# iceychris/LibreASR

Measured on AMD Instinct MI355X. Metric: audio-sec/sec/GPU (16 kHz streaming RNN-T) + p50 per-chunk latency, higher is better.
Workload: dtype f32

## Files before the change

libreasr_amd/csrc/lasr_ctx.hip.h:

```cpp
#pragma once
#include <dlfcn.h>

#include "lasr_results.hip.h"

constexpr int NW = 8;
constexpr int NCMD = 64;
constexpr int MTA = 4;

struct Cell {
    int I = 0;
    void *WxA = nullptr, *WhA = nullptr;
    void *WxC = nullptr, *WhC = nullptr;
    float *bias = nullptr, *rbias = nullptr;
    float *bn_s = nullptr, *bn_t = nullptr;
    float *h0 = nullptr, *c0 = nullptr;
    float *tab = nullptr;
};

struct lasr_ctx {
    lasr_model_desc d;
    int device = 0;
    hipStream_t stream = nullptr;
    std::string err;
    std::vector<void*> dev_allocs;
// ... 70 lines not shown
        size_t g_size = 0, ea_size = 0;
    };
    hipStream_t stream_nb = nullptr; unsigned long long* nb_done = nullptr; float* nb_buf = nullptr; size_t nb_floats = 0;
    int nb_kind = 0, nb_wgs = 0; double nb_ms = 0.0;
    hipStream_t stream_dec = nullptr;
    hipStream_t stream_lm = nullptr;
    hipEvent_t ev_lm_fork = nullptr, ev_lm_join = nullptr;
    double lm_stream_ratio[2] = {0.0, 0.0};
    int dec_stream_attempts = 0;
    double dec_stream_ratio = 0.0;
    static constexpr int NFLY = 32;
    static constexpr int RING = 64;
    static constexpr int TOKRING = 512, ENDSLOTS = 32;
    hipEvent_t ev_enc[NFLY] = {};
    hipEvent_t ev_misc = nullptr;
    int* T_row_ring[NFLY] = {};
    float* pe_ring = nullptr;
    int *c_cur = nullptr, *c_avail = nullptr, *c_iters = nullptr, *c_target = nullptr, *c_ntotal = nullptr;
    int* c_hcur_dev = nullptr;
    int *c_ntok_end = nullptr, *c_tok_ring = nullptr, *c_behind = nullptr, *c_enc_frames = nullptr, *c_enc_base = nullptr;
    int *c_done = nullptr, *c_flag_dev = nullptr;
    int* c_done2 = nullptr;
    int* c_iter = nullptr;
    std::map<std::tuple<int, int, int>, hipGraphExec_t> cgraphs;
    int* cont_host = nullptr;
    struct PendingStep { std::vector<int> rows; int Tm; int idx; bool admitted; std::vector<int> target; const int* T_row_ptr; long long serial;
                         std::vector<long long> frame_off; };
    std::vector<PendingStep> pending;
    std::vector<long long> h_frames_sub, h_fetched;
    std::vector<int> h_avail;
    std::vector<int> h_cur_seen;
    int work_left = 0;
    long long model_steps = 0, cont_iters = 0, iters_reported = 0;
    bool group_inflight = false;
    bool dec_tail_open = false;
    std::mutex mu;
    std::condition_variable cv_pump;
    std::condition_variable cv_prog;
    std::thread pump_th;
    bool pump_started = false, pump_on = false;
    std::atomic<bool> pump_stop{false};
    int pump_G = 3;
    std::atomic<long long> kick{0}, progress{0};
    int pump_rc = 0; std::string pump_err;
    int kick_n = 3, wait_n = 1;
    std::map<std::tuple<int, int, int, int, int>, hipGraphExec_t> graphs;
    bool use_graphs = true;
    bool main_graph = false;
    hipStream_t stream_cap = nullptr;
    std::map<std::vector<unsigned long long>, hipGraphExec_t> mgraphs;
    int* T_row_main = nullptr;

    struct LM {
        bool on = false;
        int E = 0, H = 0, L = 0;
        float alpha = 0.1f, theta = 1.0f, min_val = -10.0f;
        std::vector<Cell> cells;
        void* Wout = nullptr; float* bout = nullptr;
        float *ones = nullptr, *zeros = nullptr;
        std::vector<void*> h[2], y[2];
        std::vector<float*> cst[2];
        int par = 0;
        float *raw = nullptr, *lmz[2] = {nullptr, nullptr};
        int* valid[2] = {nullptr, nullptr};
        bool q8 = false;
        std::vector<void*> qWih, qWhh; void* qWout = nullptr;
        std::vector<float> s_ih, s_hh; float s_out = 0.f;
        std::vector<float*> b_ih, b_hh;
        std::vector<int> Kp_ih; int Kp_h = 0;
        float *gx = nullptr, *gh = nullptr;
        unsigned short* qa = nullptr; float* sx = nullptr;
        std::vector<unsigned short*> qh; std::vector<float*> sxh;
    } lm;

    struct Resampler { int U = 0, taps = 0, in_unit = 0; int* first = nullptr; float* w = nullptr; };
    std::map<int, Resampler> resamplers;

    int Tcap = 0;
    void *x0 = nullptr, *ybuf[2] = {nullptr, nullptr};
    float* pe_sync = nullptr;
    int tok_cap_alloc = 0;

    bool fe_fused = false;
    int ring_chunks = 0;
    std::vector<int> pend_serial;
    std::vector<char> pend_mat;
    float* win = nullptr; int* ring_pos = nullptr;
    float* pend = nullptr;
    float* stage_pcm = nullptr; size_t stage_pcm_floats = 0;
    float* win_rs = nullptr; size_t win_rs_floats = 0;
    static constexpr int NSTAGE = 64;
    hipEvent_t push_ev[NSTAGE] = {}; bool push_used[NSTAGE] = {};
    long long push_serial = 0;
    float* push_stage_host = nullptr;
    float* push_stage_host_dev = nullptr;
    float* push_stage_dev = nullptr;
    hipStream_t stream_copy = nullptr; hipEvent_t push_copied[NSTAGE] = {}; bool push_dma[NSTAGE] = {};
    struct CopyPool {
        bool init = false;
        std::vector<std::thread> th;
        std::mutex m; std::condition_variable cv;
        const char* src = nullptr; char* dst = nullptr; size_t bytes = 0, part_bytes = 0;
        const float* const* rows = nullptr; size_t row_bytes = 0;
        int parts = 0, next = 0, done = 0; long long gen = 0;
        std::atomic<long long> gen_hint{0}, done_hint{0};
        std::atomic<bool> stop{false};
    } pool;
    std::vector<int> h_ring_pos;
    struct LazyPush { bool on = false; const float* src = nullptr; std::vector<int> slots; int ev_i = -1; bool dma = false; } lazy;
    int pump_nap_pct = 0;
    int lazy_taken = 0, lazy_flushed = 0;
    bool lazy_on = true;
    float* lm_buf = nullptr; size_t lm_floats = 0;
    float* feat_stage = nullptr; size_t feat_stage_floats = 0;

    struct Cmd {
        int* T_row; int* what; int* src_idx; int* feat_sel; int* row_frames; int* token; int* emit;
        long long* row_N; long long* row_src_off; long long* row_feat_off;
    };
    char* cmd_host = nullptr; char* cmd_dev = nullptr; size_t cmd_bytes = 0; int cmd_next = 0; int cmd_inflight = 0;
    Cmd hc{}, dc{};

    int* res_host = nullptr;
    int* res_dev = nullptr;
    int* pub_arrivals = nullptr;
    size_t res_bytes = 0;

    std::vector<char> open_;
    std::vector<int> n_chunks, n_pend;
    std::vector<SlotResult> results;
    bool align_on = false;
    std::vector<long long> slot_frames;
    int* align_host = nullptr;
    int* c_frame_ring = nullptr; float* c_logp_ring = nullptr;
    struct Bias { int* block = nullptr; int n_nodes = 0; size_t n_edges = 0; bool has_back = false; int* node = nullptr; } bias;
    int* bias_pick_dev = nullptr;
    double* bias_round_dev = nullptr;

    static constexpr int NCELLEV = 64;
    bool cell_prof = false;
    bool cell_prof_events = true;
    hipEvent_t cp_ev[NCELLEV][2] = {};
    bool cp_ok = false;
    int cp_head = 0, cp_n = 0;
    int cp_cells[NCELLEV] = {};
    double cp_us = 0.0;
    long long cp_launches = 0;
    static constexpr int NCELLSLOT = 1 << 12;
    unsigned long long* cp_slots = nullptr;
    long long cp_slot_next = 0;
    std::vector<unsigned char> cp_slot_cells;
    int enc_wave = 0;
    double cp_clock_mhz = 100.0;

    static constexpr int NTRACE = 8192;
    bool tr_on = false;
    std::vector<hipEvent_t> tr_ev;
    std::vector<int> tr_tag;
    std::vector<double> tr_val;
    std::vector<int> tr_prev_cur, tr_prev_ntot;
    int tr_last_G = 0;
    hipEvent_t tr_base = nullptr;
    std::atomic<int> tr_n{0};

    struct Lattice {
        float* pp = nullptr; size_t pp_n = 0;
// ... 201 lines not shown
```

libreasr_amd/csrc/lasr_engine.hip:

```cpp
#include "lasr_host.hip.h"
#include <sys/prctl.h>
#include <time.h>

static void cont_poll(lasr_ctx* c);
static int cont_pump(lasr_ctx* c, int G);
static int pump_start(lasr_ctx* c);
static void pump_kick(lasr_ctx* c);
static int flush_lazy(lasr_ctx* c);
struct PushSrc;
static int submit_impl(lasr_ctx* c, const int* slots, int n, const PushSrc* fused, bool* fused_done);
static int push_submit_impl(lasr_ctx* c, const int* slots, int n, const float* pcm, int flags, long long* ticket, const float* const* rows);
static int overlap_probe_impl(lasr_ctx* c, int delay_us, double* ratio, hipStream_t sa = nullptr, hipStream_t sb = nullptr);
#include "lasr_prefix_tree.hip.h"
#include "lasr_bias.hip.h"
#include "lasr_cmd.hip.h"
#include "lasr_fe.hip.h"
#include "lasr_decode.hip.h"
#include "lasr_lattice_tables.hip.h"
#include "lasr_lattice.hip.h"
#include "lasr_lattice_post.hip.h"
#include "lasr_lattice_tree.hip.h"
#include "lasr_lm_score.hip.h"
#include "lasr_weights.hip.h"

// ... 248 lines not shown
            char* blk = nullptr;
            const size_t bytes = sizeof(double) * n_es + sizeof(int) * (n_tre + n_fd + n_ea) + 64;
            HIPCHK(c, hipHostMalloc((void**)&blk, bytes));
            c->host_allocs.push_back(blk);
            memset(blk, 0, bytes);
            void* dp = nullptr;
            HIPCHK(c, hipHostGetDevicePointer(&dp, blk, 0));
            char* dblk = (char*)dp;
            c->b_endsc_host = (double*)blk; c->b_endsc_dev = (double*)dblk;
            size_t off = sizeof(double) * n_es;
            c->b_tre_host = (int*)(blk + off); c->b_tre_dev = (int*)(dblk + off); off += sizeof(int) * n_tre;
            c->b_fdone_host = (int*)(blk + off); c->b_fdone_dev = (int*)(dblk + off); off += sizeof(int) * n_fd;
            c->b_endal_host = (int*)(blk + off); c->b_endal_dev = (int*)(dblk + off);
        }
    }
    RC(dalloc0(c, (char**)&c->ja, Mj * J * c->esz));
    RC(dalloc0(c, (char**)&c->cvt_a, (size_t)M * H * c->esz)); RC(dalloc0(c, (char**)&c->cvt_b, (size_t)M * H * c->esz));
    RC(dalloc0(c, &c->logits, Mj * V));
    RC(dalloc0(c, &c->ds.t_idx, M)); RC(dalloc0(c, &c->ds.iters, M)); RC(dalloc0(c, &c->ds.token, Md));
    RC(dalloc0(c, &c->ds.emit, Md)); RC(dalloc0(c, &c->ds.logp_sum, M));
    RC(dalloc0(c, &c->ds.sum_iters, M)); RC(dalloc0(c, &c->ds.n_ones, M)); RC(dalloc0(c, &c->zero_rows, M));
    RC(dalloc0(c, &c->pub_arrivals, 4));
    RC(dalloc0(c, &c->T_row_fix, M));
    RC(dalloc0(c, &c->T_row_main, M));
    {
        hipFuncAttributes fa{}, la_{};
        HIPCHK(c, hipFuncGetAttributes(&fa, (const void*)k_fe_mel<10>));
        HIPCHK(c, hipFuncGetAttributes(&la_, (const void*)k_logmel));
        const int lds_cu = 160 * 1024, excl = 98304;
        const bool wide_decode = c->Md >= 256 || lasr_ctx::LA_MAX * M >= 512;
        c->fe_lds_pad = wide_decode ? std::max(0, excl - (int)fa.sharedSizeBytes) : 0;
        if (getenv("LASR_FE_LDS_PAD")) c->fe_lds_pad = std::max(0, std::min(lds_cu - (int)fa.sharedSizeBytes, atoi(getenv("LASR_FE_LDS_PAD"))));
        c->logmel_lds_pad = c->fe_lds_pad ? std::max(0, excl - (int)la_.sharedSizeBytes) : 0;
        HIPCHK(c, hipFuncSetAttribute((const void*)k_fe_mel<10>, hipFuncAttributeMaxDynamicSharedMemorySize, lds_cu - (int)fa.sharedSizeBytes));
        HIPCHK(c, hipFuncSetAttribute((const void*)k_logmel, hipFuncAttributeMaxDynamicSharedMemorySize, lds_cu - (int)la_.sharedSizeBytes));
        HIPCHK(c, hipFuncSetAttribute((const void*)k_ln_tile, hipFuncAttributeMaxDynamicSharedMemorySize, 100 * 1024));
    }
    c->main_graph = c->bf != 0;
    if (getenv("LASR_MAIN_GRAPH")) c->main_graph = atoi(getenv("LASR_MAIN_GRAPH")) != 0;
    c->T_row_dev = c->zero_rows;
    for (int q = 0; q < lasr_ctx::NFLY; ++q) {
        RC(dalloc0(c, &c->T_row_ring[q], M));
        HIPCHK(c, hipEventCreateWithFlags(&c->ev_enc[q], hipEventDisableTiming));
    }
    HIPCHK(c, hipStreamCreateWithFlags(&c->stream_dec, hipStreamNonBlocking));
    HIPCHK(c, hipEventCreateWithFlags(&c->ev_misc, hipEventDisableTiming));
    {
        static const int pick = getenv("LASR_DEC_STREAM_PICK") ? atoi(getenv("LASR_DEC_STREAM_PICK")) : 1;
        std::vector<hipStream_t> rejected;
        c->dec_stream_attempts = 1;
        for (int attempt = 0; pick && attempt < 8; ++attempt) {
            double ratio = 0.0;
            if (overlap_probe_impl(c, 300, &ratio) != LASR_OK) { (void)hipGetLastError(); break; }
            c->dec_stream_ratio = ratio;
            if (ratio < 1.5) break;
            rejected.push_back(c->stream_dec);
            c->stream_dec = nullptr;
            HIPCHK(c, hipStreamCreateWithFlags(&c->stream_dec, hipStreamNonBlocking));
            c->dec_stream_attempts++;
        }
        for (hipStream_t st : rejected) (void)hipStreamDestroy(st);
        if (getenv("LASR_VERBOSE"))
            fprintf(stderr, "[lasr] decode stream: %d stream(s) tried, overlap probe %.2f\n", c->dec_stream_attempts, c->dec_stream_ratio);
    }
    RC(dalloc0(c, &c->pe_ring, (size_t)lasr_ctx::RING * M * J));
    RC(dalloc0(c, &c->c_cur, M)); RC(dalloc0(c, &c->c_avail, M)); RC(dalloc0(c, &c->c_iters, M)); RC(dalloc0(c, &c->c_target, M));
    RC(dalloc0(c, &c->c_ntotal, M)); RC(dalloc0(c, &c->c_enc_frames, M)); RC(dalloc0(c, &c->c_enc_base, M)); RC(dalloc0(c, &c->c_behind, 64));
    RC(dalloc0(c, &c->c_done, 64));
    RC(dalloc0(c, &c->c_done2, 64));
    RC(dalloc0(c, &c->c_iter, 4));
    HIPCHK(c, hipHostMalloc((void**)&c->cont_host, sizeof(int) * (16 + (size_t)M * (lasr_ctx::NFLY + lasr_ctx::ENDSLOTS + lasr_ctx::TOKRING))));
    memset(c->cont_host, 0, sizeof(int) * (16 + (size_t)M * (lasr_ctx::NFLY + lasr_ctx::ENDSLOTS + lasr_ctx::TOKRING)));
    {
        void* dp = nullptr;
        HIPCHK(c, hipHostGetDevicePointer(&dp, c->cont_host, 0));
        c->c_flag_dev = (int*)dp;
        c->c_hcur_dev = (int*)dp + 16;
        c->c_ntok_end = (int*)dp + 16 + (size_t)lasr_ctx::NFLY * M;
        c->c_tok_ring = c->c_ntok_end + (size_t)M * lasr_ctx::ENDSLOTS;
    }
    c->h_frames_sub.assign(M, 0); c->h_fetched.assign(M, 0); c->h_cur_seen.assign(M, 0); c->h_avail.assign(M, 0);
    c->fe_fused = M <= 512 && d.n_buffer <= 4 && d.n_stack == 10 && d.n_mels <= 128 && d.feat == 1280 && d.n_window + d.n_buffer - 1 <= 16
                  && !getenv("LASR_FE_LEGACY");
    c->h_ring_pos.assign(M, 0);
    c->ring_chunks = c->fe_fused ? d.n_window + d.n_buffer - 1 : d.n_window;
    c->pend_serial.assign((size_t)M * d.n_buffer, 0); c->pend_mat.assign((size_t)M * d.n_buffer, 0);
    RC(dalloc0(c, &c->win, (size_t)M * c->ring_chunks * d.chunk));
    RC(dalloc0(c, &c->ring_pos, M));
    RC(dalloc0(c, &c->pend, (size_t)M * d.n_buffer * d.n_stack * d.n_mels));

    lasr_ctx::Cmd tmp;
    c->cmd_bytes = cmd_layout(tmp, nullptr, M);
    HIPCHK(c, hipHostMalloc((void**)&c->cmd_host, c->cmd_bytes * NCMD));
    RC(dalloc0(c, &c->cmd_dev, c->cmd_bytes * NCMD));
    RC(ensure_T(c, std::max(d.n_buffer, 4)));

    {
        float* emb_dev = nullptr; float* EF = nullptr;
        RC(upload(c, &emb_dev, embed, (size_t)V * E));
        if (E != H) {
            Packed pk; void* wf = nullptr; float* bfn = nullptr;
            pack_tiles(pk, 0, H / 16, E, [&](int t, int ui, int k) { return ffn_w[(size_t)(16 * t + ui) * E + k]; });
            RC(upload_packed(c, &wf, pk)); RC(upload(c, &bfn, ffn_b, H));
            RC(dalloc(c, &EF, (size_t)V * H));
            GemmArgs g{}; set_operand(g, 0, emb_dev, E, 0, E / 16, wf); g.a_rows = V;
            EpiLinear::Args ea{}; ea.bias = bfn; ea.out = EF; ea.ldo = H; ea.n_rows = V; ea.t_idx = nullptr; ea.T_row = nullptr; ea.M = M;
            launch_table_gemm_f32(c, sync_view(c, c->la_sync), H / 16, V / 16, g, ea);
            HIPCHK(c, hipStreamSynchronize(c->stream));
            dfree(c, wf); dfree(c, bfn);
        } else {
            EF = emb_dev; emb_dev = nullptr;
        }
        const int G = c->G_pred;
        Packed pk; void* wt = nullptr; float* bt = nullptr;
        pack_tiles(pk, 0, G * H / 16, H, [&](int t, int ui, int k) { return in0_w[(size_t)(16 * t + ui) * H + k]; });
        RC(upload_packed(c, &wt, pk)); RC(upload(c, &bt, in0_b.data(), in0_b.size()));
        RC(dalloc(c, &c->pred[0].tab, (size_t)V * G * H));
        GemmArgs g{}; set_operand(g, 0, EF, H, 0, H / 16, wt); g.a_rows = V;
        EpiLinear::Args ea{}; ea.bias = bt; ea.out = c->pred[0].tab; ea.ldo = G * H; ea.n_rows = V; ea.t_idx = nullptr; ea.T_row = nullptr; ea.M = M;
        launch_table_gemm_f32(c, sync_view(c, c->la_sync), G * H / 16, V / 16, g, ea);
        HIPCHK(c, hipStreamSynchronize(c->stream));
        HIPCHK(c, hipGetLastError());
        dfree(c, wt); dfree(c, bt); dfree(c, EF); dfree(c, emb_dev);
    }

    c->open_.assign(M, 0); c->n_chunks.assign(M, 0); c->n_pend.assign(M, 0);
    c->results.assign(M, SlotResult{}); c->slot_frames.assign(M, 0);
    c->ev_ok = true;
    for (auto& e : c->ev)
        if (hipEventCreate(&e) != hipSuccess) c->ev_ok = false;
    static const int bos_cache = getenv("LASR_BOS_CACHE") ? atoi(getenv("LASR_BOS_CACHE")) : 1;
    if (bos_cache && c->W == 1) {
        RC(cmd_begin(c));
        c->hc.what[0] = 2;
        RC(cmd_commit(c));
        RC(apply_reset(c, sync_view(c, c->la_sync), true));
        BosArgs b{};
        b.H = H; b.J = J; b.Lp = d.pred_layers; b.M = M; b.lstm = d.pred_cell; b.bf = c->bf;
        c->bos_h.assign(d.pred_layers, nullptr); c->bos_c.assign(d.pred_layers, nullptr);
        for (int l = 0; l < d.pred_layers; ++l) {
            RC(dalloc(c, &c->bos_h[l], H));
            if (d.pred_cell) RC(dalloc(c, &c->bos_c[l], H));
            b.pred_h[l] = c->pred_h[c->pred_par][l]; b.pred_c[l] = d.pred_cell ? c->pred_c[0][l] : nullptr;
            b.bos_h[l] = c->bos_h[l]; b.bos_c[l] = c->bos_c[l];
        }
        RC(dalloc(c, &c->bos_pp, J));
        b.pp = c->pp[0]; b.bos_pp = c->bos_pp;
        hipLaunchKernelGGL(k_bos_capture, dim3(grid1(std::max(H, J))), dim3(256), 0, c->stream, b);
        HIPCHK(c, hipStreamSynchronize(c->stream));
        HIPCHK(c, hipGetLastError());
        c->bos_ready = true;
    }
    return LASR_OK;
}

int lasr_create(int device, const lasr_model_desc* d, const float* weights, size_t n_weights, void* hip_stream,
                lasr_ctx** out) {
    if (!out) return LASR_EINVAL;
    *out = nullptr;
    lasr_ctx* c = new lasr_ctx();
    if (!valid_desc(d)) { int rc = fail(c, LASR_EINVAL, "invalid model description"); *out = c; return rc; }
    c->d = *d;
    c->device = device;
    *out = c;
    if (!weights || n_weights != lasr_weight_count(d))
        return fail(c, LASR_EINVAL, "weight blob has %zu floats, expected %zu", n_weights, lasr_weight_count(d));
// ... 2378 lines not shown

int lasr_overlap_probe(lasr_ctx* c, int delay_us, double* ratio) {
    if (!c || !ratio || delay_us < 1 || delay_us > 1000000) return c ? fail(c, LASR_EINVAL, "bad argument") : LASR_EINVAL;
    RC(flush_lazy(c));
    RC(require_idle(c));
    HIPCHK(c, hipSetDevice(c->device));
    return overlap_probe_impl(c, delay_us, ratio);
}
static int overlap_probe_impl(lasr_ctx* c, int delay_us, double* ratio, hipStream_t sa, hipStream_t sb) {
    if (!sb) { sa = c->stream; sb = c->stream_dec; }
    hipEvent_t e0, e1, e2;
    HIPCHK(c, hipEventCreate(&e0)); HIPCHK(c, hipEventCreate(&e1)); HIPCHK(c, hipEventCreate(&e2));
    const unsigned long long ticks = (unsigned long long)delay_us * 100ull;
    for (int rep = 0; rep < 2; ++rep) {
        HIPCHK(c, hipEventRecord(e0, sa));
        HIPCHK(c, hipStreamWaitEvent(sb, e0, 0));
        hipLaunchKernelGGL(k_delay, dim3(1), dim3(64), 0, sa, rep ? ticks : 100ull);
        hipLaunchKernelGGL(k_delay, dim3(1), dim3(64), 0, sb, rep ? ticks : 100ull);
        HIPCHK(c, hipEventRecord(e2, sb));
        HIPCHK(c, hipStreamWaitEvent(sa, e2, 0));
        HIPCHK(c, hipEventRecord(e1, sa));
        HIPCHK(c, hipEventSynchronize(e1));
    }
    float ms = 0.f;
    HIPCHK(c, hipEventElapsedTime(&ms, e0, e1));
    (void)hipEventDestroy(e0); (void)hipEventDestroy(e1); (void)hipEventDestroy(e2);
    *ratio = 1e3 * (double)ms / (double)delay_us;
    return LASR_OK;
}

int lasr_bench_neighbour(lasr_ctx* c, int kind, int n_wg, int ms, double* rate) {
    if (!c || kind < 0 || kind > 4) return c ? fail(c, LASR_EINVAL, "bad argument") : LASR_EINVAL;
    HIPCHK(c, hipSetDevice(c->device));
    if (kind == 0) {
        if (rate) *rate = 0.0;
        if (!c->stream_nb || !c->nb_kind) return LASR_OK;
        HIPCHK(c, hipStreamSynchronize(c->stream_nb));
        std::vector<unsigned long long> done(c->nb_wgs);
        HIPCHK(c, hipMemcpy(done.data(), c->nb_done, sizeof(unsigned long long) * c->nb_wgs, hipMemcpyDeviceToHost));
        double total = 0.0;
        for (auto v : done) total += (double)v;
        if (rate) *rate = c->nb_kind == 1 ? total * 2048.0 / (c->nb_ms * 1e-3) * 1e-12 : total * 1024.0 / (c->nb_ms * 1e-3) * 1e-9;
        c->nb_kind = 0;
        return LASR_OK;
    }
    if (n_wg < 1 || n_wg > 4096 || ms < 1 || ms > 5000) return fail(c, LASR_EINVAL, "neighbour: 1..4096 workgroups, 1..5000 ms");
    if (c->nb_kind) return fail(c, LASR_ESTATE, "a neighbour is already running: collect it with kind 0");
    if (!c->stream_nb) {
        std::vector<hipStream_t> rejected;
        for (int attempt = 0; attempt < 8 && !c->stream_nb; ++attempt) {
            hipStream_t st = nullptr;
            HIPCHK(c, hipStreamCreateWithFlags(&st, hipStreamNonBlocking));
            double r0 = 0.0, r1 = 0.0;
            if (overlap_probe_impl(c, 300, &r0, c->stream, st) != LASR_OK || overlap_probe_impl(c, 300, &r1, c->stream_dec, st) != LASR_OK) {
                (void)hipGetLastError(); rejected.push_back(st); break;
            }
            if (r0 < 1.5 && r1 < 1.5) c->stream_nb = st; else rejected.push_back(st);
        }
        for (hipStream_t st : rejected) (void)hipStreamDestroy(st);
        if (!c->stream_nb) return fail(c, LASR_EHIP, "no hardware queue left for the neighbour stream");
        RC(dalloc(c, &c->nb_done, 4096));
        c->nb_floats = (size_t)128 << 20;
        RC(dalloc0(c, &c->nb_buf, c->nb_floats));
        HIPCHK(c, hipDeviceSynchronize());
    }
    HIPCHK(c, hipMemsetAsync(c->nb_done, 0, sizeof(unsigned long long) * 4096, c->stream_nb));
    const unsigned long long ticks = (unsigned long long)ms * 100000ull;
    if (kind == 1) hipLaunchKernelGGL(k_nb_mfma, dim3(n_wg), dim3(64), 0, c->stream_nb, ticks, c->nb_done, c->nb_buf);
    else if (kind == 2) hipLaunchKernelGGL(k_nb_load, dim3(n_wg), dim3(64), 0, c->stream_nb, ticks, (const f32x4*)c->nb_buf, c->nb_floats / 4, (size_t)0, 0, c->nb_done, c->nb_buf);
    else if (kind == 3) hipLaunchKernelGGL(k_nb_load, dim3(n_wg), dim3(64), 0, c->stream_nb, ticks, (const f32x4*)c->nb_buf, c->nb_floats / 4, (size_t)(96 << 10) / 16, 1, c->nb_done, c->nb_buf);
    else hipLaunchKernelGGL(k_nb_load, dim3(n_wg), dim3(64), 0, c->stream_nb, ticks, (const f32x4*)c->nb_buf, (size_t)(128 << 20) / 16, (size_t)0, 1, c->nb_done, c->nb_buf);
    HIPCHK(c, hipGetLastError());
    c->nb_kind = kind; c->nb_wgs = n_wg; c->nb_ms = (double)ms;
    return LASR_OK;
}

int lasr_debug_config(lasr_ctx* c, const char* key, int* value) {
    if (!c || !key || !value) return LASR_EINVAL;
    const struct { const char* k; int v; } tab[] = {
        {"enc_wave", c->enc_wave}, {"enc_u12", (int)c->enc_u12}, {"main_graph", (int)c->main_graph},
        {"pump_G", c->pump_G}, {"la_stream", c->la_stream}, {"la_offline", c->la_offline},
        {"cell_nw", c->cell_nw ? c->cell_nw : (c->bf ? 8 : 4)}, {"use_graphs", (int)c->use_graphs}, {"M", c->M},
        {"push_lazy", (int)c->lazy_on}, {"pump_nap_pct", c->pump_nap_pct}, {"lazy_taken", c->lazy_taken}, {"lazy_flushed", c->lazy_flushed},
        {"fe_lds_pad", c->fe_lds_pad}, {"roctx", roctx_state().push != nullptr ? 1 : 0},
        {"lat_R", LAT_R}, {"lat_umax", LAT_UMAX},
        {"lat_enc_us", c->lat.us[0]}, {"lat_pred_us", c->lat.us[1]}, {"lat_blocks_us", c->lat.us[2]}, {"lat_dp_us", c->lat.us[3]},
        {"lat_band_wmax", LAT_BAND_WMAX}, {"lat_band_umax", LAT_BAND_UMAX}, {"lat_bp_words", LAT_BP_WORDS},
        {"lat_post_us", c->lat.us[4]},
    };
    for (const auto& e : tab)
        if (!strcmp(e.k, key)) { *value = e.v; return LASR_OK; }
    return fail(c, LASR_EINVAL, "lasr_debug_config: unknown key '%s'", key);
}

int lasr_bench_cell(lasr_ctx* c, int layer, int iters, double* us) {
    if (!c || !us || layer < 0 || layer >= c->d.enc_layers || iters < 1) return c ? fail(c, LASR_EINVAL, "bad argument") : LASR_EINVAL;
    HIPCHK(c, hipSetDevice(c->device));
    const int Tn = 1;
    RC(ensure_T(c, Tn));
    const int H = c->d.hidden, I = c->enc[layer].I, M = c->M;
    hipLaunchKernelGGL(k_fill_rand, dim3(grid1((size_t)c->Tcap * M * I)), dim3(256), 0, c->stream, layer == 0 ? c->x0 : c->ybuf[(layer - 1) & 1],
                       (size_t)c->Tcap * M * I, 17u, c->bf);
    for (int p = 0; p < 2; ++p)
        hipLaunchKernelGGL(k_fill_rand, dim3(grid1((size_t)M * H)), dim3(256), 0, c->stream, c->enc_h[p][layer], (size_t)M * H, 23u + p, c->bf);
    RC(cmd_begin(c));
    for (int r = 0; r < c->d.max_streams; ++r) c->hc.T_row[r] = Tn;
    RC(cmd_commit(c));
    RC(commit_T_rows(c, Tn));
    const void* xsrc = layer == 0 ? c->x0 : c->ybuf[(layer - 1) & 1];
    const int mt_total = c->Tcap * c->MT;
    auto one = [&]() { launch_enc_cell(c, c->stream, layer, 0, xsrc, mt_total, c->ybuf[layer & 1], mt_total); c->enc_par ^= 1; };
    for (int i = 0; i < 3; ++i) one();
    hipEvent_t e0, e1;
    HIPCHK(c, hipEventCreate(&e0)); HIPCHK(c, hipEventCreate(&e1));
    HIPCHK(c, hipEventRecord(e0, c->stream));
    for (int i = 0; i < iters; ++i) one();
    HIPCHK(c, hipEventRecord(e1, c->stream));
    HIPCHK(c, hipEventSynchronize(e1));
    float ms = 0.f;
    HIPCHK(c, hipEventElapsedTime(&ms, e0, e1));
    (void)hipEventDestroy(e0); (void)hipEventDestroy(e1);
    *us = (double)ms * 1000.0 / ((double)iters * Tn);
    c->cmd_inflight = 0;
    HIPCHK(c, hipGetLastError());
    return LASR_OK;
}

}

#include "lasr_front.hip.h"

#include "lasr_band_windows.hip.h"
#include "lasr_lattice_band.hip.h"
#include "lasr_lattice_band_post.hip.h"
extern "C" {
int lasr_band_windows(int T, int U, int band, const int32_t* frames, const int32_t* lo_cur, int32_t* lo_out, int* touch) {
    return lasr_bw::band_windows(T, U, band, frames, lo_cur, lo_out, touch);
}
int lasr_align_band_pcm(lasr_ctx* c, const int* slots, int n, const float* pcm, const int64_t* n_samples, const int32_t* tokens,
                        const int32_t* n_tokens, int band, int max_passes, const int32_t* lo_in, double* loglik, double* viterbi,
                        int32_t* frames, float* logps, float* blank_lp, float* emit_lp, int32_t* lo_out, int32_t* passes, int32_t* touch) {
    LatCall k;
    const LatBandIO io{band, max_passes, lo_in, lo_out, passes, touch, &k};
    const AlignCall a{slots, n, tokens, n_tokens, LatOut{loglik, viterbi, frames, logps, blank_lp, emit_lp}, nullptr, &io};
    return align_impl(c, a, OfflineAudio{pcm, n_samples, nullptr});
}
int lasr_align_band_feats(lasr_ctx* c, const int* slots, int n, const float* feats, const int32_t* n_frames, const int32_t* tokens,
                          const int32_t* n_tokens, int band, int max_passes, const int32_t* lo_in, double* loglik, double* viterbi,
                          int32_t* frames, float* logps, float* blank_lp, float* emit_lp, int32_t* lo_out, int32_t* passes, int32_t* touch) {
    LatCall k;
    const LatBandIO io{band, max_passes, lo_in, lo_out, passes, touch, &k};
    const AlignCall a{slots, n, tokens, n_tokens, LatOut{loglik, viterbi, frames, logps, blank_lp, emit_lp}, nullptr, &io};
    return align_impl(c, a, OfflineAudio{feats, nullptr, n_frames});
}
int lasr_align_band_post_pcm(lasr_ctx* c, const int* slots, int n, const float* pcm, const int64_t* n_samples, const int32_t* tokens,
                             const int32_t* n_tokens, int band, int max_passes, const int32_t* lo_in, double* loglik, double* viterbi,
                             int32_t* frames, float* logps, float* blank_lp, float* emit_lp, int32_t* lo_out, int32_t* passes, int32_t* touch,
                             float* occ_blank, float* occ_emit, double* tok_mean, double* tok_var, int32_t* tok_peak_frame, double* tok_peak) {
    LatCall k;
    const LatBandIO io{band, max_passes, lo_in, lo_out, passes, touch, &k};
    const LatPostOut p{nullptr, nullptr, occ_blank, occ_emit, tok_mean, tok_var, tok_peak_frame, tok_peak};
    const AlignCall a{slots, n, tokens, n_tokens, LatOut{loglik, viterbi, frames, logps, blank_lp, emit_lp}, lat_post_any(p) ? &p : nullptr, &io};
    return align_impl(c, a, OfflineAudio{pcm, n_samples, nullptr});
}
int lasr_align_band_post_feats(lasr_ctx* c, const int* slots, int n, const float* feats, const int32_t* n_frames, const int32_t* tokens,
                               const int32_t* n_tokens, int band, int max_passes, const int32_t* lo_in, double* loglik, double* viterbi,
                               int32_t* frames, float* logps, float* blank_lp, float* emit_lp, int32_t* lo_out, int32_t* passes, int32_t* touch,
// ... 50 lines not shown
```

libreasr_amd/csrc/lasr_fe.hip.h:

```cpp
#pragma once

namespace {

template <class A>
void fill_mel_consts(const lasr_ctx* c, A& m) {
    const lasr_model_desc& d = c->d;
    m.window = c->window; m.tw512 = c->tw512; m.tw1024 = c->tw1024; m.fb_start = c->fb_start; m.fb_off = c->fb_off;
    m.fb_w = c->fb_w; m.n_mels = d.n_mels; m.hop = d.hop;
    m.win_off = (d.n_fft - d.win) / 2; m.win_len = d.win; m.fb_nnz = c->fb_nnz;
}

int stream_frame0(const lasr_ctx* c, int* nf_out) {
    const lasr_model_desc& d = c->d;
    const long long N = (long long)d.n_window * d.chunk;
    const int T = 1 + (int)(N / d.hop);
    const int a0 = T / 3 + 1;
    if (nf_out) *nf_out = std::min(d.n_stack, T - a0);
    return a0;
}
int stream_window_fault(const lasr_ctx* c, int* nf_out = nullptr) {
    int nf = 0;
    (void)stream_frame0(c, &nf);
    if (nf_out) *nf_out = nf;
    if (nf < c->d.n_stack) return 1;
    return (long long)c->d.n_window * c->d.chunk <= c->d.n_fft / 2 ? 2 : 0;
}

void launch_logmel_ring(lasr_ctx* c, MelArgs& m) {
    const lasr_model_desc& d = c->d;
    fill_mel_consts(c, m);
    m.pcm = c->win; m.N = (long long)d.n_window * d.chunk; m.stream = 1; m.ring_head = c->ring_pos; m.chunk = d.chunk;
    m.n_window = d.n_window; m.ring_chunks = c->ring_chunks; m.frame0 = stream_frame0(c, nullptr);
    m.frames_per_row = d.n_stack; m.out = c->pend; m.out_frames = d.n_buffer * d.n_stack;
    hipLaunchKernelGGL(k_logmel, dim3((d.n_stack + 3) / 4, c->M), dim3(256), c->logmel_lds_pad, c->stream, m);
}
void launch_logmel_window(lasr_ctx* c, MelArgs& m, const float* pcm, long long N, int frame0, int n) {
    const lasr_model_desc& d = c->d;
    fill_mel_consts(c, m);
    m.pcm = pcm; m.N = N; m.stream = 0; m.by_value = 1; m.frame0 = frame0; m.frames_per_row = d.n_stack;
    m.out = c->pend; m.out_frames = d.n_buffer * d.n_stack; m.chunk = d.chunk; m.n_window = d.n_window;
    hipLaunchKernelGGL(k_logmel, dim3((d.n_stack + 3) / 4, n), dim3(256), 0, c->stream, m);
}
void launch_logmel_offline(lasr_ctx* c, const float* pcm, long long N, int rows, int T, float* out, const long long* row_N = nullptr,
                           const long long* row_src_off = nullptr, const int* row_frames = nullptr) {
    const lasr_model_desc& d = c->d;
    MelArgs m{};
    fill_mel_consts(c, m);
    m.pcm = pcm; m.N = N; m.stream = 0;
    m.ring_head = nullptr; m.chunk = d.chunk; m.n_window = d.n_window; m.row_sel = nullptr; m.frame0 = 0;
    m.frames_per_row = T; m.out = out; m.out_frames = T;
    m.row_N = row_N; m.row_src_off = row_src_off; m.row_frames = row_frames;
    hipLaunchKernelGGL(k_logmel, dim3((T + 3) / 4, rows), dim3(256), 0, c->stream, m);
}

void fill_fe_mel_args(const lasr_ctx* c, FeMelArgs& m, float* pend) {
    const lasr_model_desc& d = c->d;
    fill_mel_consts(c, m);
    m.pcm = c->win; m.ring_pos = c->ring_pos; m.chunk = d.chunk; m.n_window = d.n_window; m.ring_chunks = c->ring_chunks;
    m.frame0 = stream_frame0(c, nullptr);
    m.pend = pend; m.pend_frames = d.n_buffer * d.n_stack;
    for (int r = 0; r < 512; ++r) { m.idx[r] = -1; m.tp_pk[r] = 0; m.age_pk[r] = 0; }
}
void launch_fe_mel(lasr_ctx* c, const FeMelArgs& m) {
    hipLaunchKernelGGL((k_fe_mel<10>), dim3(2 * c->d.n_buffer, c->M), dim3(320), c->fe_lds_pad, c->stream, m);
}

void launch_stack_ln(lasr_ctx* c, int mode, const float* src, int src_frames, int frame_step, const long long* row_off,
                     const int* T_row, int Tmax) {
    const lasr_model_desc& d = c->d;
    StackLnArgs a{};
    a.src = src; a.mode = mode; a.src_frames = src_frames; a.frame_step = frame_step; a.row_off = row_off;
    a.T_row = T_row; a.ln_w = c->ln_w; a.ln_b = c->ln_b; a.x0 = c->x0; a.F = d.feat; a.n_mels = d.n_mels;
    a.n_stack = d.n_stack; a.M = c->M; a.MT = c->MT; a.mt_total = c->Tcap * c->MT; a.feats_out = nullptr; a.bf = c->bf; a.Tmax = Tmax;
    const dim3 grid((Tmax + 3) / 4, c->M), block(256);
    if (a.F == 1280 && a.n_stack == 10) hipLaunchKernelGGL((k_stack_ln<20, 10>), grid, block, 0, c->stream, a);
    else hipLaunchKernelGGL((k_stack_ln<32, 0>), grid, block, 0, c->stream, a);
}
void stack_ln_logmel(lasr_ctx* c, const float* logmel, int src_frames, int frame_step, const int* T_row, int Tmax) {
    launch_stack_ln(c, 0, logmel, src_frames, frame_step, nullptr, T_row, Tmax);
}
void stack_ln_feats(lasr_ctx* c, const float* feats, const long long* row_off, const int* T_row, int Tmax) {
    launch_stack_ln(c, 1, feats, 0, 0, row_off, T_row, Tmax);
}

void launch_ln_tile(lasr_ctx* c, int Tm) {
    const lasr_model_desc& d = c->d;
    LnTileArgs t{};
    t.pend = c->pend; t.pend_frames = d.n_buffer * d.n_stack; t.T_row = c->T_row_dev; t.ln_w = c->ln_w; t.ln_b = c->ln_b;
    t.x0 = c->x0; t.MT = c->MT; t.mt_total = c->Tcap * c->MT; t.bf = c->bf;
    constexpr int ln_z = 4;
    hipLaunchKernelGGL(k_ln_tile, dim3(c->MT, Tm, ln_z), dim3(1024), c->fe_lds_pad ? 98304 : 16 * 1284 * 4, c->stream, t);
}

}
```

libreasr_amd/csrc/lasr_kernels.hip.h:

```cpp
#pragma once
#include <hip/hip_runtime.h>
#include <stdint.h>
#include <type_traits>

#include "lasr_beamhist.hip.h"
#include "lasr_beam_merge.hip.h"

namespace lasr {

typedef float f32x4 __attribute__((ext_vector_type(4)));

__device__ __forceinline__ float sigmoid_(float x) { return 1.0f / (1.0f + expf(-x)); }

#include "lasr_gemm.hip.h"

struct AvailV { int v[512]; };
template <class Avail>
__device__ __forceinline__ void ja_body(const float* __restrict__ pe, const float* __restrict__ pp, const int* __restrict__ t_idx,
                                        const Avail& avail, bool lim, int* __restrict__ avail_out, void* __restrict__ ja, int J,
                                        int M, int MT, int ring, int bf, int W, int M_enc, int la) {
    const int idx = blockIdx.x * blockDim.x + threadIdx.x;
    if (idx >= M * J) return;
    const int r = idx / J, j = idx - r * J;
    const int q = W > 1 ? r / W : r;
// ... 1454 lines not shown
    __shared__ float s_fbw[1536];
    __shared__ int s_fbs[128], s_fbo[129];
    __shared__ float2 s_tw512[512], s_tw1024[513];
    const int w = threadIdx.x >> 6, j = threadIdx.x & 63;
    const MelTables tab{s_fbw, s_fbs, s_fbo, s_tw512, s_tw1024};
    stage_mel_tables(tab, a.tw512, a.tw1024, a.fb_w, a.fb_start, a.fb_off, a.fb_nnz, a.n_mels);
    int fidx = blockIdx.x * 4 + w;
    const int row = blockIdx.y;
    int n_frames = a.frames_per_row;
    long long N = a.N;
    if (a.row_frames) {
        n_frames = a.row_frames[row];
        if (n_frames <= 0) return;
        N = a.row_N[row];
    }
    const bool valid = fidx < n_frames;
    if (!valid) fidx = n_frames - 1;
    int out_frame = fidx;
    int t = fidx;
    const float* src = a.pcm;
    int head = 0;
    const int NR = a.ring_chunks > 0 ? a.ring_chunks : a.n_window;
    if (a.stream) {
        if (a.by_value && a.trow_out && blockIdx.x == 0 && threadIdx.x == 0) a.trow_out[row] = a.trow_v[row];
        const int sel = a.by_value ? (int)a.sel_v[row] : a.row_sel[row];
        if (sel < 0) return;
        out_frame = sel + fidx;
        t = a.frame0 + fidx;
        head = (a.ring_head[row] - (a.by_value ? (int)a.age_v[row] : 0) - a.n_window + 2 * NR) % NR;
        src = a.pcm + (size_t)row * NR * a.chunk;
    } else if (a.row_frames) {
        src = a.pcm + a.row_src_off[row];
    } else {
        src = a.pcm + (size_t)row * a.N;
        if (a.by_value) { out_frame = (int)a.sel_v[row] + fidx; t = a.frame0 + fidx; }
    }
    const int out_row = (!a.stream && a.by_value) ? (int)a.dst_row_v[row] : row;
    const long long base = (long long)t * a.hop - 512;
    auto sample = [&](int n) -> float {
        const float wv = (n < a.win_off || n >= a.win_off + a.win_len) ? 0.f : a.window[n];
        long long q = base + n;
        if (q < 0) q = -q;
        if (q >= N) q = 2 * (N - 1) - q;
        float x;
        if (a.stream) {
            const int qi = (int)q;
            const int ck = qi / a.chunk, wi = qi - ck * a.chunk;
            int slot = head + ck;
            if (slot >= NR) slot -= NR;
            x = src[(size_t)slot * a.chunk + wi];
        } else {
            x = src[q];
        }
        return x * wv;
    };
    cf v[8];
#pragma unroll
    for (int m = 0; m < 8; ++m) {
        const int n = j + 64 * m;
        v[m] = cf{sample(2 * n), sample(2 * n + 1)};
    }
    fft1024_power(v, sz[w], sp[w], s_tw512, s_tw1024, j);
    if (!valid) return;
    mel_log(sp[w], tab, a.n_mels, j, a.out + ((size_t)out_row * a.out_frames + out_frame) * a.n_mels);
}

struct FeMelArgs {
    const float* window; const float2* tw512; const float2* tw1024;
    const int* fb_start; const int* fb_off; const float* fb_w;
    int n_mels, hop, fb_nnz, win_off, win_len;
    float* pcm;
    int* ring_pos;
    int chunk, n_window, ring_chunks, frame0;
    float* pend;
    int pend_frames;
    int* trow_out;
    int* enc_frames;
    int* enc_base;
    const float* src;
    const float* src2;
    short idx[512];
    unsigned char tp_pk[512];
    unsigned short age_pk[512];
};
template <int NSTACK>
__global__ __launch_bounds__(32 * NSTACK) void k_fe_mel(const FeMelArgs a) {
    constexpr int NWV = NSTACK / 2;
    __shared__ float2 sz[NWV][512 + 8];
    __shared__ float sp[NWV][520];
    __shared__ float s_fbw[1536];
    __shared__ int s_fbs[128], s_fbo[129];
    __shared__ float2 s_tw512[512], s_tw1024[513];
    const int w = threadIdx.x >> 6, j = threadIdx.x & 63;
    const int tp = blockIdx.x >> 1, half = blockIdx.x & 1, row = blockIdx.y;
    const int Tr = a.tp_pk[row] & 15, pos = a.tp_pk[row] >> 4;
    const int si = a.src ? (int)a.idx[row] : -1;
    const int NR = a.ring_chunks;
    const bool two = si >= 0 && a.src2 != nullptr;
    const int pos_new = two ? (pos + 1) % NR : pos;
    if (blockIdx.x == 0) {
        if (threadIdx.x == 0) {
            a.trow_out[row] = Tr;
            if (a.enc_frames) { const int e = a.enc_frames[row]; a.enc_base[row] = e; a.enc_frames[row] = e + Tr; }
            if (si >= 0) a.ring_pos[row] = (pos_new + 1) % NR;
        }
        if (si >= 0) {
            for (int q = two ? 0 : 1; q < 2; ++q) {
                float* d = a.pcm + ((size_t)row * NR + (q ? pos_new : pos)) * a.chunk;
                const float* s = (q ? a.src : a.src2) + (size_t)si * a.chunk;
                if ((a.chunk & 3) == 0 && ((((uintptr_t)s) | ((uintptr_t)d)) & 15) == 0) {
                    for (int i = threadIdx.x; i < a.chunk / 4; i += blockDim.x) ((float4*)d)[i] = ((const float4*)s)[i];
                } else {
                    for (int i = threadIdx.x; i < a.chunk; i += blockDim.x) d[i] = s[i];
                }
            }
        }
    }
    if (tp >= Tr) return;
    const int age = (a.age_pk[row] >> (4 * tp)) & 15;
    if (age == 15) return;
    const MelTables tab{s_fbw, s_fbs, s_fbo, s_tw512, s_tw1024};
    stage_mel_tables(tab, a.tw512, a.tw1024, a.fb_w, a.fb_start, a.fb_off, a.fb_nnz, a.n_mels);
    const int f = half * NWV + w;
    const int pos_after = si >= 0 ? (pos_new + 1) % NR : pos;
    const int head = (pos_after - age - a.n_window + 2 * NR) % NR;
    const float* ring = a.pcm + (size_t)row * NR * a.chunk;
    const float* fresh = si >= 0 ? a.src + (size_t)si * a.chunk : nullptr;
    const float* fresh2 = two ? a.src2 + (size_t)si * a.chunk : nullptr;
    const int N = a.n_window * a.chunk;
    const int base = (a.frame0 + f) * a.hop - 512;
    auto sample = [&](int n) -> float {
        const float wv = (n < a.win_off || n >= a.win_off + a.win_len) ? 0.f : a.window[n];
        int q = base + n;
        if (q < 0) q = -q;
        if (q >= N) q = 2 * (N - 1) - q;
        int ck = 0, wi = q;
        while (wi >= a.chunk) { wi -= a.chunk; ++ck; }
        int slot = head + ck;
        if (slot >= NR) slot -= NR;
        const float x = (fresh && slot == pos_new) ? fresh[wi] : (fresh2 && slot == pos) ? fresh2[wi] : ring[(size_t)slot * a.chunk + wi];
        return x * wv;
    };
    cf v[8];
#pragma unroll
    for (int m = 0; m < 8; ++m) {
        const int n = j + 64 * m;
        v[m] = cf{sample(2 * n), sample(2 * n + 1)};
    }
    fft1024_power(v, sz[w], sp[w], s_tw512, s_tw1024, j);
    mel_log(sp[w], tab, a.n_mels, j, a.pend + ((size_t)row * a.pend_frames + (size_t)tp * NSTACK + f) * a.n_mels);
}

inline __global__ void k_resample(const float* __restrict__ x, long long N_in, const int* __restrict__ first,
                           const float* __restrict__ w, int U, int taps, int in_unit, float* __restrict__ out,
                           long long N_out) {
    const long long n = (long long)blockIdx.x * blockDim.x + threadIdx.x;
    if (n >= N_out) return;
    const float* xr = x + (size_t)blockIdx.y * N_in;
    const int ph = (int)(n % U);
    const long long start = first[ph] + (n / U) * in_unit;
    const float* wp = w + (size_t)ph * taps;
    float acc = 0.f;
    for (int j = 0; j < taps; ++j) {
        const long long i = start + j;
        if (i >= 0 && i < N_in) acc += wp[j] * xr[i];
    }
    out[(size_t)blockIdx.y * N_out + n] = acc;
}

inline __global__ void k_stack(const float* __restrict__ logmel, int T_frames, int n_mels, int n_stack, int stride,
                        float* __restrict__ feats, int Tp, int F) {
    const int tp = blockIdx.x, row = blockIdx.y;
    const float* lm = logmel + (size_t)row * T_frames * n_mels;
    float* o = feats + ((size_t)row * Tp + tp) * F;
    for (int f = threadIdx.x; f < F; f += blockDim.x) {
        const int m = f / n_stack, k = f - m * n_stack;
        o[f] = lm[(size_t)(stride * tp + k) * n_mels + m];
    }
}

struct StackLnArgs {
    const float* src;
    int mode;
    int src_frames;
    int frame_step;
    const long long* row_off;
    const int* T_row;
    const float* ln_w;
    const float* ln_b;
    void* x0;
    int F, n_mels, n_stack, M, MT, mt_total, bf;
    float* feats_out;
    int Tmax;
};
template <int VPL, int NSTACK = 0>
__global__ __launch_bounds__(256) void k_stack_ln(const StackLnArgs a) {
    const int w = threadIdx.x >> 6, lane = threadIdx.x & 63;
    const int tp = blockIdx.x * 4 + w, row = blockIdx.y;
    if (tp >= a.T_row[row]) return;
    float x[VPL];
    float sum = 0.f;
    const int n_stack = NSTACK > 0 ? NSTACK : a.n_stack;
#pragma unroll
    for (int q = 0; q < VPL; ++q) {
        const int f = lane + 64 * q;
        float val = 0.f;
        if (NSTACK == 0 && f >= a.F) {
        } else if (a.mode == 0) {
            const int m = f / n_stack, k = f - m * n_stack;
            val = a.src[((size_t)row * a.src_frames + (size_t)a.frame_step * tp + k) * a.n_mels + m];
        } else {
            val = a.src[(size_t)(a.row_off[row] + tp) * a.F + f];
        }
        x[q] = val;
        sum += val;
    }
#pragma unroll
    for (int o = 32; o > 0; o >>= 1) sum += __shfl_xor(sum, o);
    const float mu = sum / (float)a.F;
    float var = 0.f;
#pragma unroll
    for (int q = 0; q < VPL; ++q) {
        const float d = (lane + 64 * q < a.F) ? x[q] - mu : 0.f;
        var += d * d;
    }
#pragma unroll
    for (int o = 32; o > 0; o >>= 1) var += __shfl_xor(var, o);
    const float rstd = 1.0f / sqrtf(var / (float)a.F + 1e-5f);
#pragma unroll
    for (int q = 0; q < VPL; ++q) {
        const int f = lane + 64 * q;
        if (f >= a.F) continue;
        if (a.feats_out) a.feats_out[((size_t)row * a.Tmax + tp) * a.F + f] = x[q];
        const float y = (x[q] - mu) * rstd * a.ln_w[f] + a.ln_b[f];
        act_st(a.bf, a.x0, act_off(a.bf, tp * a.MT * 16 + row, f, a.mt_total), y);
// ... 94 lines not shown
```

Before: 58040.

## Fuse mel frontend and layer-norm tiling into one kernel launch

Adds a k_fe_mel_ln kernel in which one block computes all ten stacked mel frames of a time step, then applies layer norm and writes the encoder input tile (fp32 or bf16) directly. This replaces the two-block-per-timestep mel kernel plus the separate ln_tile kernel, removing one launch and the round trip through the pend buffer for normalization. Global sample loads are issued before the mel tables are staged into LDS, so their latency can overlap. Blocks are larger (640 threads, more LDS), which may lower occupancy. The path is enabled by default when fused FE is active, no LDS pad is set and n_mels is 128, and it can be turned off with LASR_FE_ONE=0.

```diff
diff --git a/libreasr_amd/csrc/lasr_ctx.hip.h b/libreasr_amd/csrc/lasr_ctx.hip.h
--- a/libreasr_amd/csrc/lasr_ctx.hip.h
+++ b/libreasr_amd/csrc/lasr_ctx.hip.h
@@ -176,6 +176,7 @@
     int tok_cap_alloc = 0;
 
     bool fe_fused = false;
+    bool fe_one = false;
     int ring_chunks = 0;
     std::vector<int> pend_serial;
     std::vector<char> pend_mat;
diff --git a/libreasr_amd/csrc/lasr_engine.hip b/libreasr_amd/csrc/lasr_engine.hip
--- a/libreasr_amd/csrc/lasr_engine.hip
+++ b/libreasr_amd/csrc/lasr_engine.hip
@@ -354,6 +354,7 @@
     c->h_frames_sub.assign(M, 0); c->h_fetched.assign(M, 0); c->h_cur_seen.assign(M, 0); c->h_avail.assign(M, 0);
     c->fe_fused = M <= 512 && d.n_buffer <= 4 && d.n_stack == 10 && d.n_mels <= 128 && d.feat == 1280 && d.n_window + d.n_buffer - 1 <= 16
                   && !getenv("LASR_FE_LEGACY");
+    c->fe_one = fe_one_launch(c);
     c->h_ring_pos.assign(M, 0);
     c->ring_chunks = c->fe_fused ? d.n_window + d.n_buffer - 1 : d.n_window;
     c->pend_serial.assign((size_t)M * d.n_buffer, 0); c->pend_mat.assign((size_t)M * d.n_buffer, 0);
@@ -2898,7 +2899,7 @@
         {"pump_G", c->pump_G}, {"la_stream", c->la_stream}, {"la_offline", c->la_offline},
         {"cell_nw", c->cell_nw ? c->cell_nw : (c->bf ? 8 : 4)}, {"use_graphs", (int)c->use_graphs}, {"M", c->M},
         {"push_lazy", (int)c->lazy_on}, {"pump_nap_pct", c->pump_nap_pct}, {"lazy_taken", c->lazy_taken}, {"lazy_flushed", c->lazy_flushed},
-        {"fe_lds_pad", c->fe_lds_pad}, {"roctx", roctx_state().push != nullptr ? 1 : 0},
+        {"fe_lds_pad", c->fe_lds_pad}, {"fe_one", (int)c->fe_one}, {"roctx", roctx_state().push != nullptr ? 1 : 0},
         {"lat_R", LAT_R}, {"lat_umax", LAT_UMAX},
         {"lat_enc_us", c->lat.us[0]}, {"lat_pred_us", c->lat.us[1]}, {"lat_blocks_us", c->lat.us[2]}, {"lat_dp_us", c->lat.us[3]},
         {"lat_band_wmax", LAT_BAND_WMAX}, {"lat_band_umax", LAT_BAND_UMAX}, {"lat_bp_words", LAT_BP_WORDS},
diff --git a/libreasr_amd/csrc/lasr_fe.hip.h b/libreasr_amd/csrc/lasr_fe.hip.h
--- a/libreasr_amd/csrc/lasr_fe.hip.h
+++ b/libreasr_amd/csrc/lasr_fe.hip.h
@@ -60,8 +60,17 @@
     m.frame0 = stream_frame0(c, nullptr);
     m.pend = pend; m.pend_frames = d.n_buffer * d.n_stack;
     for (int r = 0; r < 512; ++r) { m.idx[r] = -1; m.tp_pk[r] = 0; m.age_pk[r] = 0; }
+    m.ln_w = c->ln_w; m.ln_b = c->ln_b; m.x0 = c->x0; m.MT = c->MT; m.mt_total = c->Tcap * c->MT; m.bf = c->bf;
+}
+bool fe_one_launch(const lasr_ctx* c) {
+    if (!c->fe_fused || c->fe_lds_pad != 0 || c->d.n_mels != 128) return false;
+    return !(getenv("LASR_FE_ONE") && atoi(getenv("LASR_FE_ONE")) == 0);
 }
 void launch_fe_mel(lasr_ctx* c, const FeMelArgs& m) {
+    if (c->fe_one) {
+        hipLaunchKernelGGL((k_fe_mel_ln<10>), dim3(c->d.n_buffer, c->M), dim3(640), 0, c->stream, m);
+        return;
+    }
     hipLaunchKernelGGL((k_fe_mel<10>), dim3(2 * c->d.n_buffer, c->M), dim3(320), c->fe_lds_pad, c->stream, m);
 }
 
@@ -84,6 +93,7 @@
 }
 
 void launch_ln_tile(lasr_ctx* c, int Tm) {
+    if (c->fe_one) return;
     const lasr_model_desc& d = c->d;
     LnTileArgs t{};
     t.pend = c->pend; t.pend_frames = d.n_buffer * d.n_stack; t.T_row = c->T_row_dev; t.ln_w = c->ln_w; t.ln_b = c->ln_b;
diff --git a/libreasr_amd/csrc/lasr_kernels.hip.h b/libreasr_amd/csrc/lasr_kernels.hip.h
--- a/libreasr_amd/csrc/lasr_kernels.hip.h
+++ b/libreasr_amd/csrc/lasr_kernels.hip.h
@@ -1560,6 +1560,9 @@
     short idx[512];
     unsigned char tp_pk[512];
     unsigned short age_pk[512];
+    const float* ln_w; const float* ln_b;
+    void* x0;
+    int MT, mt_total, bf;
 };
 template <int NSTACK>
 __global__ __launch_bounds__(32 * NSTACK) void k_fe_mel(const FeMelArgs a) {
@@ -1629,6 +1632,129 @@
     mel_log(sp[w], tab, a.n_mels, j, a.pend + ((size_t)row * a.pend_frames + (size_t)tp * NSTACK + f) * a.n_mels);
 }
 
+template <int NSTACK>
+__global__ __launch_bounds__(64 * NSTACK) void k_fe_mel_ln(const FeMelArgs a) {
+    constexpr int NM = 128, F = NM * NSTACK, NQ = F / 64;
+    __shared__ float2 sz[NSTACK][512 + 8];
+    __shared__ float sp[NSTACK][520];
+    __shared__ float s_fbw[1536];
+    __shared__ int s_fbs[128], s_fbo[129];
+    __shared__ float2 s_tw512[512], s_tw1024[513];
+    __shared__ float xs[F];
+    const int w = threadIdx.x >> 6, j = threadIdx.x & 63;
+    const int tp = blockIdx.x, row = blockIdx.y;
+    const int Tr = a.tp_pk[row] & 15, pos = a.tp_pk[row] >> 4;
+    const int si = a.src ? (int)a.idx[row] : -1;
+    const int NR = a.ring_chunks;
+    const bool two = si >= 0 && a.src2 != nullptr;
+    const int pos_new = two ? (pos + 1) % NR : pos;
+    const int age = tp < Tr ? (a.age_pk[row] >> (4 * tp)) & 15 : 15;
+    const bool compute = age != 15;
+    auto side_duties = [&] {
+        if (threadIdx.x == 0) {
+            a.trow_out[row] = Tr;
+            if (a.enc_frames) { const int e = a.enc_frames[row]; a.enc_base[row] = e; a.enc_frames[row] = e + Tr; }
+            if (si >= 0) a.ring_pos[row] = (pos_new + 1) % NR;
+        }
+        if (si >= 0) {
+            for (int q = two ? 0 : 1; q < 2; ++q) {
+                float* d = a.pcm + ((size_t)row * NR + (q ? pos_new : pos)) * a.chunk;
+                const float* s = (q ? a.src : a.src2) + (size_t)si * a.chunk;
+                if ((a.chunk & 3) == 0 && ((((uintptr_t)s) | ((uintptr_t)d)) & 15) == 0) {
+                    for (int i = threadIdx.x; i < a.chunk / 4; i += blockDim.x) ((float4*)d)[i] = ((const float4*)s)[i];
+                } else {
+                    for (int i = threadIdx.x; i < a.chunk; i += blockDim.x) d[i] = s[i];
+                }
+            }
+        }
+    };
+    if (blockIdx.x == 0 && !compute) side_duties();
+    if (tp >= Tr) return;
+    const int EPL = a.bf ? 8 : 4;
+    const bool storer = (int)threadIdx.x < F / EPL;
+    float lw[8], lb[8];
+#pragma unroll
+    for (int e = 0; e < 8; ++e) {
+        const bool on = storer && e < EPL;
+        lw[e] = on ? a.ln_w[threadIdx.x * EPL + e] : 0.f;
+        lb[e] = on ? a.ln_b[threadIdx.x * EPL + e] : 0.f;
+    }
+    float* pf = a.pend + ((size_t)row * a.pend_frames + (size_t)tp * NSTACK + w) * NM;
+    float m0, m1;
+    if (compute) {
+        const int pos_after = si >= 0 ? (pos_new + 1) % NR : pos;
+        const int head = (pos_after - age - a.n_window + 2 * NR) % NR;
+        const float* ring = a.pcm + (size_t)row * NR * a.chunk;
+        const float* fresh = si >= 0 ? a.src + (size_t)si * a.chunk : nullptr;
+        const float* fresh2 = two ? a.src2 + (size_t)si * a.chunk : nullptr;
+        const int N = a.n_window * a.chunk;
+        const int base = (a.frame0 + w) * a.hop - 512;
+        auto sample_ld = [&](int n, float& x, float& wv) {
+            wv = (n < a.win_off || n >= a.win_off + a.win_len) ? 0.f : a.window[n];
+            int q = base + n;
+            if (q < 0) q = -q;
+            if (q >= N) q = 2 * (N - 1) - q;
+            int ck = 0, wi = q;
+            while (wi >= a.chunk) { wi -= a.chunk; ++ck; }
+            int slot = head + ck;
+            if (slot >= NR) slot -= NR;
+            x = (fresh && slot == pos_new) ? fresh[wi] : (fresh2 && slot == pos) ? fresh2[wi] : ring[(size_t)slot * a.chunk + wi];
+        };
+        float sx[16], sw[16];
+#pragma unroll
+        for (int m = 0; m < 8; ++m) {
+            const int n = j + 64 * m;
+            sample_ld(2 * n, sx[2 * m], sw[2 * m]);
+            sample_ld(2 * n + 1, sx[2 * m + 1], sw[2 * m + 1]);
+        }
+        if (blockIdx.x == 0) side_duties();
+        const MelTables tab{s_fbw, s_fbs, s_fbo, s_tw512, s_tw1024};
+        stage_mel_tables(tab, a.tw512, a.tw1024, a.fb_w, a.fb_start, a.fb_off, a.fb_nnz, a.n_mels);
+        cf v[8];
+#pragma unroll
+        for (int m = 0; m < 8; ++m) v[m] = cf{sx[2 * m] * sw[2 * m], sx[2 * m + 1] * sw[2 * m + 1]};
+        fft1024_power(v, sz[w], sp[w], s_tw512, s_tw1024, j);
+        float* fr = (float*)sz[w];
+        mel_log(sp[w], tab, a.n_mels, j, fr);
+        wave_sync_lds();
+        m0 = fr[j]; m1 = fr[j + 64];
+        pf[j] = m0; pf[j + 64] = m1;
+    } else {
+        m0 = pf[j]; m1 = pf[j + 64];
+    }
+    xs[j * NSTACK + w] = m0; xs[(j + 64) * NSTACK + w] = m1;
+    __syncthreads();
+    float x[NQ];
+    float sum = 0.f;
+#pragma unroll
+    for (int q = 0; q < NQ; ++q) { x[q] = xs[j + 64 * q]; sum += x[q]; }
+#pragma unroll
+    for (int o = 32; o > 0; o >>= 1) sum += __shfl_xor(sum, o);
+    const float mu = sum / (float)F;
+    float var = 0.f;
+#pragma unroll
+    for (int q = 0; q < NQ; ++q) { const float d = x[q] - mu; var += d * d; }
+#pragma unroll
+    for (int o = 32; o > 0; o >>= 1) var += __shfl_xor(var, o);
+    const float rstd = 1.0f / sqrtf(var / (float)F + 1e-5f);
+    if (!storer) return;
+    const int c = threadIdx.x >> 2, g = threadIdx.x & 3;
+    const size_t at = ((size_t)c * a.mt_total + (size_t)tp * a.MT + (row >> 4)) * 64 + g * 16 + (row & 15);
+    float y[8];
+#pragma unroll
+    for (int e = 0; e < 8; ++e) y[e] = e < EPL ? (xs[threadIdx.x * EPL + e] - mu) * rstd * lw[e] + lb[e] : 0.f;
+    if (!a.bf) {
+        ((float4*)a.x0)[at] = float4{y[0], y[1], y[2], y[3]};
+    } else {
+        uint4 o;
+        o.x = (unsigned)f32_to_bf16(y[0]) | ((unsigned)f32_to_bf16(y[1]) << 16);
+        o.y = (unsigned)f32_to_bf16(y[2]) | ((unsigned)f32_to_bf16(y[3]) << 16);
+        o.z = (unsigned)f32_to_bf16(y[4]) | ((unsigned)f32_to_bf16(y[5]) << 16);
+        o.w = (unsigned)f32_to_bf16(y[6]) | ((unsigned)f32_to_bf16(y[7]) << 16);
+        ((uint4*)a.x0)[at] = o;
+    }
+}
+
 inline __global__ void k_resample(const float* __restrict__ x, long long N_in, const int* __restrict__ first,
                            const float* __restrict__ w, int U, int taps, int in_unit, float* __restrict__ out,
                            long long N_out) {
```

New measurement: 57900. About the same (-0.2%).
